# Layr-Labs/rust-kzg-bn254

Hardware: AMD Instinct MI355X
Metric: G1-MSM (scalar,point) pairs/s = 2^20 x KZG coeff-form commitments/s, 2^20-point SRS (higher is better)
Workload: dtype int32x9 (29-bit limbs, 64-bit accumulate); 1 GPU; G1 MSM 2^20 scalars (KZG::commit_coeff_form), scalars resident in HBM; step k commits buffer k mod 8 (8 distinct resident scalar sets, 256 MiB); pipeline_depth=2, steps_per_launch=1

## Files before the change

rust-kzg-bn254_amd/csrc/msm.hip:

```cpp
#include "engine.h"
#include <new>
#include "msm_kernels.h"
#include "host_msm_epilogue.h"
#include "host_pairing.h"

#include <algorithm>
#include <cstdlib>
#include <chrono>
#include <cstdio>
#include <cstring>
#include <type_traits>
#include <vector>

namespace kzg {

void MsmWorkspace::release() {
    DeviceBuffer* all[] = {&scalars, &bases, &bases_wire, &digits, &sorted, &count, &blockbase, &sort_tmp, &sort_key, &sort_small, &offs, &block_sums,
                           &head, &cont, &blob, &bucket, &chunkS, &chunkTmp, &chunkA, &out_wire};
    for (auto* b : all) b->release();
    if (pinned_out) { (void)hipHostFree(pinned_out); pinned_out = nullptr; }
    if (ev_ready) { for (auto& e : ev) (void)hipEventDestroy(e); ev_ready = false; }
    if (ev_done) { (void)hipEventDestroy(ev_done); ev_done = nullptr; }
    if (ev_sorted) { (void)hipEventDestroy(ev_sorted); ev_sorted = nullptr; }
}
// ... 127 lines not shown
    const Plan& p = L.p;
    MsmWorkspace& ws = L.ws;
    hipStream_t st = L.st;
    const uint32_t n_total = p.n * p.batch;
    KZG_HIP_TRY(L.ctx, hipMemsetAsync(ws.count.p, 0, (size_t)p.G * 4, st));
    hipLaunchKernelGGL(k_msm_digits, dim3((n_total + 255) / 256), dim3(256), 0, st, L.d_scalars, n_total, p.n, p.c, p.W, ws.digits.as<uint32_t>(), (uint32_t*)nullptr);
    KZG_MARK(1);
    if (p.sort_small) {
        const uint32_t entries = (uint32_t)p.entries(), ge = (uint32_t)((p.entries() + 255) / 256);
        KZG_HIP_TRY(L.ctx, hipMemsetAsync(ws.blockbase.p, 0, (size_t)p.G * 4, st));
        hipLaunchKernelGGL(k_sort_small_hist, dim3(ge), dim3(256), 0, st, ws.digits.as<uint32_t>(), entries, p.set_len, p.B, ws.count.as<uint32_t>());
        scan_counts(L);
        KZG_MARK(2);
        hipLaunchKernelGGL(k_sort_small_scatter, dim3(ge), dim3(256), 0, st, ws.digits.as<uint32_t>(), entries, p.n, p.set_len, p.B,
                           ws.offs.as<uint32_t>(), ws.blockbase.as<uint32_t>(), p.idx_stride, (uint32_t)p.W, ws.sorted.as<uint32_t>());
    } else {
        const size_t lds_bytes = (size_t)p.B * 4;
        hipLaunchKernelGGL(k_sort_hist, dim3(p.tiles), dim3(256), lds_bytes, st, ws.digits.as<uint32_t>(), p.set_len, p.tile_len,
                           p.tiles_per_set, p.B, ws.count.as<uint32_t>(), ws.blockbase.as<uint32_t>());
        scan_counts(L);
        KZG_MARK(2);
        hipLaunchKernelGGL(k_sort_scatter, dim3(p.tiles), dim3(256), lds_bytes, st, ws.digits.as<uint32_t>(), p.n, p.set_len, p.tile_len,
                           p.tiles_per_set, p.B, ws.offs.as<uint32_t>(), ws.blockbase.as<uint32_t>(), p.idx_stride,
                           (uint32_t)p.W, ws.sorted.as<uint32_t>());
    }
    KZG_MARK(3);
    return KZG_OK;
}

static int32_t enqueue_sort(const Launch& L, const PolyPtrs* poly_ptrs) {
    const Plan& p = L.p;
    kzg_ctx* ctx = L.ctx;
    MsmWorkspace& ws = L.ws;
    if (p.bitsum) {
        for (int i = 0; i <= 4; ++i) KZG_MARK(i);
        return KZG_OK;
    }
    { int32_t rc = set_sort_lds_attributes(ctx); if (rc != KZG_OK) return rc; }
    const bool stagger = p.tables && p.polys >= 2;
    if (stagger && ctx->last_sorted && ctx->last_sorted_stream != L.st) KZG_HIP_TRY(ctx, hipStreamWaitEvent(L.st, ctx->last_sorted, 0));
    KZG_MARK(0);
    const uint32_t clean_g = ws.count_zero_ptr == ws.count.p ? ws.count_zero_g : 0;
    ws.count_zero_g = 0;
    const int32_t rc = p.sort2 ? sort_two_level(L, poly_ptrs) : p.lean_sort ? sort_lean(L, clean_g) : sort_from_digits(L);
    if (rc != KZG_OK) return rc;
    KZG_MARK(4);
    if (p.tables) {
        if (!ws.ev_sorted) KZG_HIP_TRY(ctx, hipEventCreateWithFlags(&ws.ev_sorted, hipEventDisableTiming));
        KZG_HIP_TRY(ctx, hipEventRecord(ws.ev_sorted, L.st));
        ctx->last_sorted = ws.ev_sorted;
        ctx->last_sorted_stream = L.st;
    }
    return KZG_OK;
}

static int32_t enqueue_accumulate(const Launch& L) {
    const Plan& p = L.p;
    MsmWorkspace& ws = L.ws;
    if (!p.bitsum && !p.fused)
        dispatch<true, false>(!L.bases.identity_free, [&](auto identity_bases) {
            hipLaunchKernelGGL(k_msm_accumulate<decltype(identity_bases)::value>, dim3(p.nl / 256), dim3(256), 0, L.st, L.bases.points, ws.sorted.as<uint32_t>(),
                               ws.offs.as<uint32_t>(), p.G, ws.head.as<int32_t>(), (size_t)p.G, ws.cont.as<int32_t>(), (size_t)p.nl, p.idx_log, p.stride_adj);
        });
    KZG_MARK(5);
    return KZG_OK;
}

static int32_t reduce_bitsum(const Launch& L) {
    const Plan& p = L.p;
    dispatch<8, 16, 32>(p.bitsum_chunk, [&](auto chunk) {
        hipLaunchKernelGGL(k_bitsum_level1<decltype(chunk)::value>, dim3(p.bitsum_wg), dim3(256), 0, L.st, L.bases.points, L.bases.table_stride, L.d_scalars, p.n,
                           L.ws.chunkS.as<int32_t>());
    });
    KZG_MARK(6);
    hipLaunchKernelGGL(k_bitsum_level2, dim3(p.n_out), dim3(256), 0, L.st, L.ws.chunkS.as<int32_t>(), p.bitsum_wg, L.d_out);
    return KZG_OK;
}

static int32_t reduce_tables(const Launch& L) {
    const Plan& p = L.p;
    MsmWorkspace& ws = L.ws;
    const uint32_t G1 = p.G1(), G1p = p.G1p();
    int32_t* x1 = ws.chunkS.as<int32_t>();
    dispatch<true, false>(p.quad1, [&](auto quads) {
        using LG = std::conditional_t<decltype(quads)::value, QuadLanes, PairLanes>;
        if (p.fused)
            hipLaunchKernelGGL(k_msm_bucket_bits1_fused<LG>, dim3(G1), dim3(LG::THREADS), 0, L.st, L.bases.points, ws.sorted.as<uint32_t>(), ws.offs.as<uint32_t>(), p.B,
                               p.idx_log, p.stride_adj, G1, x1, (size_t)7 * G1, L.d_out);
        else
            hipLaunchKernelGGL(k_msm_bucket_bits1<LG>, dim3(G1), dim3(LG::THREADS), 0, L.st, ws.offs.as<uint32_t>(), p.B, p.nl, ws.head.as<int32_t>(), (size_t)p.G,
                               ws.cont.as<int32_t>(), (size_t)p.nl, G1, x1, (size_t)7 * G1, L.d_out);
    });
    KZG_MARK(6);
    if (p.polys && p.c == 7) {
        hipLaunchKernelGGL(k_batch_finish, dim3((p.polys + 63) / 64), dim3(64), 0, L.st, x1, (size_t)7 * G1, G1, L.d_out);
    } else if (G1 > 1) {
        const uint32_t waves2 = 7 * G1p;
        if (p.quad)
            hipLaunchKernelGGL(k_red_bits2q, dim3(waves2), dim3(256), 0, L.st, x1, (size_t)7 * G1, G1, G1p, L.d_out);
        else
            hipLaunchKernelGGL(k_red_bits2p, dim3((waves2 + 1) / 2), dim3(128), 0, L.st, x1, (size_t)7 * G1, G1, G1p, L.d_out);
    }
    return KZG_OK;
}

static int32_t reduce_generic(const Launch& L) {
    const Plan& p = L.p;
    MsmWorkspace& ws = L.ws;
    hipStream_t st = L.st;
    const uint32_t n_chunks = p.n_chunks(), n_windows = p.n_windows();
    const uint32_t gg = (p.G + 255) / 256;
    hipLaunchKernelGGL(k_msm_bucket_fin, dim3(gg), dim3(256), 0, st, ws.offs.as<uint32_t>(), p.G, p.nl, p.m, n_chunks, ws.head.as<int32_t>(), (size_t)p.G,
                       ws.cont.as<int32_t>(), (size_t)p.nl, ws.bucket.as<int32_t>(), (size_t)p.G);
    const uint32_t gc = (n_chunks + 255) / 256;
    KZG_MARK(6);
    hipLaunchKernelGGL(k_red_chunk_sums, dim3(gc), dim3(256), 0, st, ws.bucket.as<int32_t>(), (size_t)p.G, n_chunks, p.m,
                       ws.chunkS.as<int32_t>(), (size_t)n_chunks);
    hipLaunchKernelGGL(k_red_suffix_scan, dim3(n_windows), dim3(p.T), 0, st, ws.chunkS.as<int32_t>(), ws.chunkTmp.as<int32_t>(),
                       (size_t)n_chunks, p.T);
    hipLaunchKernelGGL(k_red_chunk_running, dim3(gc), dim3(256), 0, st, ws.bucket.as<int32_t>(), (size_t)p.G,
                       ws.chunkS.as<int32_t>(), (size_t)n_chunks, n_chunks, p.T, p.m, ws.chunkA.as<int32_t>());
    hipLaunchKernelGGL(k_red_window_sum, dim3(n_windows), dim3(p.T), 0, st, ws.chunkA.as<int32_t>(), (size_t)n_chunks, p.T,
                       L.d_out);
    return KZG_OK;
}

static int32_t enqueue_reduce(const Launch& L) {
    const int32_t rc = L.p.bitsum ? reduce_bitsum(L) : L.p.tables ? reduce_tables(L) : reduce_generic(L);
    if (rc != KZG_OK) return rc;
    KZG_MARK(7);
    return KZG_OK;
}
#undef KZG_MARK

static PlanContext plan_context(const kzg_ctx* ctx) {
    PlanContext pc;
    pc.msm_c_override = ctx->msm_c_override;
    pc.msm_seg_override = ctx->msm_seg_override;
    pc.reduction_lanes = ctx->reduction_lanes;
    pc.acc_wave_slots = ctx->acc_wave_slots;
    for (int sl = 0; sl < KZG_NUM_SLOTS; ++sl) pc.other_in_flight |= ctx->slot_pending[sl] != nullptr;
    return pc;
}

static int32_t msm_enqueue(kzg_ctx* ctx, MsmWorkspace& ws, hipStream_t st, const MsmBases& bases, const uint4* d_scalars, size_t n,
                           uint32_t batch, Pending* pend, uint32_t out_off = 0, uint32_t out_cap = MSM_MAX_OUT, uint32_t polys = 0,
                           const PolyPtrs* poly_ptrs = nullptr) {
    const Plan p = make_plan(plan_context(ctx), n, bases, batch, polys);
    {
        const char* error = nullptr;
        const int32_t rc = msm_plan_status(p, bases, polys, out_off, out_cap, &error);
        if (error) ctx->last_error = error;
        if (rc != KZG_OK) return rc;
    }
    DeviceBuffer* const buffers[WS_BUFFERS] = {&ws.digits, &ws.sorted, &ws.count, &ws.sort_tmp, &ws.sort_key, &ws.sort_small, &ws.blockbase, &ws.offs, &ws.block_sums,
                                               &ws.head, &ws.cont, &ws.bucket, &ws.chunkS, &ws.chunkTmp, &ws.chunkA};
    for (int i = 0; i < WS_BUFFERS; ++i) KZG_HIP_TRY(ctx, buffers[i]->reserve(p.bytes[i]));
    if (!ws.pinned_out) {
        KZG_HIP_TRY(ctx, hipHostMalloc(&ws.pinned_out, (size_t)MSM_MAX_OUT * 32 * 4 + MSM_MAX_PARTS * 4, hipHostMallocDefault));
        KZG_HIP_TRY(ctx, hipHostGetDevicePointer(&ws.pinned_out_dev, ws.pinned_out, 0));
    }
    const Launch L{ctx, ws, st, bases, d_scalars, p, reinterpret_cast<uint32_t*>(ws.pinned_out_dev) + (size_t)out_off * 32, ctx->profiling};
    if (L.prof && !ws.ev_ready) {
        for (auto& e : ws.ev) KZG_HIP_TRY(ctx, hipEventCreate(&e));
        ws.ev_ready = true;
    }
    int32_t rc;
    RoctxPhases phases;
    phases.begin(p.bitsum ? "kzg:msm:bit sums" : "kzg:msm:sort");
    if ((rc = enqueue_sort(L, poly_ptrs)) != KZG_OK) return rc;
    if (!p.bitsum) phases.begin("kzg:msm:accumulate");
    if ((rc = enqueue_accumulate(L)) != KZG_OK) return rc;
    if (!p.bitsum) phases.begin("kzg:msm:bucket reduction");
    if ((rc = enqueue_reduce(L)) != KZG_OK) return rc;
    phases.end();
// ... 281 lines not shown
```

rust-kzg-bn254_amd/csrc/msm_kernels.h:

```cpp
#pragma once
#include <hip/hip_runtime.h>
#include "curve_pair.h"
#include "curve_quad.h"
#include "naf.h"
#include "msm_limits.h"

namespace kzg {

__device__ __forceinline__ void latency_bound_kernel() {
#if !defined(KZG_NO_SETPRIO)
    __builtin_amdgcn_s_setprio(3);
#endif
}

constexpr uint32_t DIGIT_NONE = 0xFFFFFFFFu;

__global__ void __launch_bounds__(256)
k_msm_digits(const uint4* __restrict__ scalars, uint32_t n_total, uint32_t n, int c, int W, uint32_t* __restrict__ digits,
             uint32_t* __restrict__ count = nullptr ) {
    latency_bound_kernel();
    uint32_t j = blockIdx.x * blockDim.x + threadIdx.x;
    if (j >= n_total) return;
    const uint32_t msm = j / n, i = j - msm * n;
    uint4 lo = scalars[2 * (size_t)j], hi = scalars[2 * (size_t)j + 1];
    uint32_t w32[8] = {lo.x, lo.y, lo.z, lo.w, hi.x, hi.y, hi.z, hi.w};
    uint32_t k[8];
    fe_wire_to_canonical_words<FrParams>(k, w32);
    const uint32_t mask = (1u << c) - 1u, half = 1u << (c - 1);
    uint32_t carry = 0;
    for (int w = 0; w < W; ++w) {
        uint32_t raw = (k[0] & mask) + carry;
#pragma unroll
        for (int j = 0; j < 7; ++j) k[j] = (k[j] >> c) | (k[j + 1] << (32 - c));
        k[7] >>= c;
        uint32_t neg = raw > half;
        uint32_t mag = neg ? (1u << c) - raw : raw;
        carry = neg;
        uint32_t v = DIGIT_NONE;
        if (mag != 0) {
            v = (mag - 1) | (neg << 31);
            if (count) atomicAdd(&count[mag - 1], 1u);
        }
        digits[((size_t)msm * W + w) * n + i] = v;
    }
}


template <int T>
__device__ __forceinline__ uint32_t block_excl_scan(uint32_t v, uint32_t* total, uint32_t* lds ) {
    const int t = threadIdx.x;
    lds[t] = v;
    __syncthreads();
    for (int d = 1; d < T; d <<= 1) {
        uint32_t x = (t >= d) ? lds[t - d] : 0u;
        __syncthreads();
        lds[t] += x;
        __syncthreads();
    }
    uint32_t incl = lds[t];
    *total = lds[T - 1];
    __syncthreads();
    return incl - v;
}
__device__ __forceinline__ uint4 scan1_load(const uint32_t* __restrict__ count, uint32_t g, uint32_t hi) {
    if (g + 4 <= hi) return *reinterpret_cast<const uint4*>(count + g);
    uint4 v = make_uint4(0, 0, 0, 0);
    if (g < hi) v.x = count[g];
    if (g + 1 < hi) v.y = count[g + 1];
    if (g + 2 < hi) v.z = count[g + 2];
    return v;
}
template <bool LEAN>
__global__ void __launch_bounds__(SCAN1_THREADS)
k_scan_counts_1wg(uint32_t* __restrict__ count, uint32_t G, uint32_t* __restrict__ offs , uint32_t* __restrict__ cursor ) {
    latency_bound_kernel();
    __shared__ uint32_t wave_total[SCAN1_THREADS / 64];
    const uint32_t t = threadIdx.x, w = t >> 6, lane = t & 63;
    const uint32_t per_wave = (((G + SCAN1_THREADS / 64 - 1) / (SCAN1_THREADS / 64)) + 255u) & ~255u;
    const uint32_t lo = min(G, w * per_wave), hi = min(G, lo + per_wave);
    uint32_t s = 0;
    for (uint32_t g0 = lo; g0 < hi; g0 += 1024) {
        const uint32_t g = g0 + lane * 4;
        const uint4 a = scan1_load(count, g, hi), b = scan1_load(count, g + 256, hi), c = scan1_load(count, g + 512, hi), d = scan1_load(count, g + 768, hi);
        s += a.x + a.y + a.z + a.w + b.x + b.y + b.z + b.w + c.x + c.y + c.z + c.w + d.x + d.y + d.z + d.w;
    }
    for (int d = 32; d >= 1; d >>= 1) s += __shfl_xor(s, d, 64);
    if (lane == 0) wave_total[w] = s;
    __syncthreads();
// ... 983 lines not shown
__device__ __forceinline__ void bucket_partial_lanes(typename LG::Point& v, const BucketSpan& s, uint32_t k, const int32_t* __restrict__ head, size_t head_stride,
                                                     const int32_t* __restrict__ cont, size_t cont_stride, typename LG::Role role) {
    if (k == 0) { LG::load(v, head, head_stride, s.g, role); return; }
    LG::load(v, cont, cont_stride, bucket_cont_lane(s, k), role);
}
template <class LG>
__device__ __noinline__ void bucket_sum_heavy(typename LG::Point& tot, uint32_t g, uint32_t t1, uint32_t np, uint32_t long_run, uint32_t lane,
                                              const int32_t* __restrict__ head, size_t head_stride, const int32_t* __restrict__ cont, size_t cont_stride) {
    const uint32_t grp = lane / LG::LANES;
    const typename LG::Role role = LG::role(lane);
    BucketSpan h;
    h.g = g; h.t1 = t1; h.np = np; h.long_run = long_run != 0;
    typename LG::Point part;
    LG::set_inf(part);
    const uint32_t loads = (np + LG::GROUPS - 1) / LG::GROUPS;
#pragma unroll 1
    for (uint32_t step = 0; step < loads + LG::LOG_GROUPS; ++step) {
        typename LG::Point u;
        bool on;
        if (step < loads) {
            const uint32_t k = grp + LG::GROUPS * step;
            on = k < np;
            if (on) bucket_partial_lanes<LG>(u, h, k, head, head_stride, cont, cont_stride, role);
        } else {
            const uint32_t d = (LG::GROUPS / 2) >> (step - loads);
            LG::shfl_down(u, part, (int)(LG::LANES * d));
            on = grp < d;
        }
        if (on) {
            typename LG::Point r;
            LG::add(r, part, u, role);
            part = r;
        }
    }
    LG::shfl(tot, part, (int)(lane & (LG::LANES - 1)));
}
template <class LG>
__device__ __forceinline__ void bucket_sum_lanes(typename LG::Point& acc, const BucketSpan& s, uint32_t lane, typename LG::Role role, const int32_t* __restrict__ head,
                                                 size_t head_stride, const int32_t* __restrict__ cont, size_t cont_stride) {
    LG::set_inf(acc);
    const bool heavy = s.np > NP_SERIAL;
    if (!heavy) {
#pragma unroll 1
        for (uint32_t k = 0; k < s.np; ++k) {
            typename LG::Point v, r;
            bucket_partial_lanes<LG>(v, s, k, head, head_stride, cont, cont_stride, role);
            LG::add(r, acc, v, role);
            acc = r;
        }
    }
    unsigned long long todo = __ballot(heavy && (lane & (LG::LANES - 1)) == 0);
    while (todo) {
        const int src = __ffsll((long long)todo) - 1;
        todo &= todo - 1;
        typename LG::Point tot;
        bucket_sum_heavy<LG>(tot, __shfl(s.g, src, 64), __shfl(s.t1, src, 64), __shfl(s.np, src, 64), (uint32_t)__shfl((int)s.long_run, src, 64), lane,
                             head, head_stride, cont, cont_stride);
        if ((int)(lane & ~(LG::LANES - 1)) == src) acc = tot;
    }
}
template <class LG>
__global__ void __launch_bounds__(LG::THREADS) __attribute__((amdgpu_waves_per_eu(LG::WAVES, LG::WAVES)))
k_msm_bucket_bits1(const uint32_t* __restrict__ offs, uint32_t B, uint32_t nl, const int32_t* __restrict__ head, size_t head_stride,
                   const int32_t* __restrict__ cont, size_t cont_stride, uint32_t G1, int32_t* __restrict__ x1, size_t x_stride,
                   uint32_t* __restrict__ out_wire ) {
    latency_bound_kernel();
    __shared__ int32_t lds[LG::ZETA_LDS_WORDS];
    const uint32_t g = blockIdx.x, w = threadIdx.x >> 6, lane = threadIdx.x & 63, gp = w * LG::GROUPS + lane / LG::LANES;
    const typename LG::Role role = LG::role(lane);
    const uint32_t L = acc_seg_len(offs[B], nl);
    const uint32_t bkt = g * 64 + gp;
    BucketSpan s;
    s.g = bkt; s.t1 = 0; s.np = 0; s.long_run = false;
    if (bkt < B && L) s = bucket_span(offs, bkt, L);
    typename LG::Point v;
    bucket_sum_lanes<LG>(v, s, lane, role, head, head_stride, cont, cont_stride);
    LG::zeta64(v, lane, w, role, lds);
    const int zr = zeta_role(gp);
    if (zr < 0) return;
    if (G1 == 1) LG::store_wire(out_wire, (size_t)zr, v, role);
    else LG::store(x1, x_stride, (size_t)zr * G1 + g, v, role);
}
template <class LG>
__device__ __noinline__ void fused_heavy_bucket(typename LG::Point& tot, uint32_t hb, uint32_t he, uint32_t lane, const uint4* __restrict__ points,
                                                const uint32_t* __restrict__ sorted, uint32_t idx_log, uint32_t stride_adj) {
    const uint32_t grp = lane / LG::LANES;
    const typename LG::Role role = LG::role(lane);
    typename LG::Point part;
    LG::set_inf(part);
#pragma unroll 1
    for (uint32_t e = hb + grp; e < he; e += LG::GROUPS) {
        const uint32_t cur = sorted[e];
        const uint4* src = points + 4 * acc_point_index(cur & 0x7FFFFFFFu, idx_log, stride_adj) + LG::affine_half(role);
        const uint4 q0 = src[0], q1 = src[1];
        const uint32_t w32[8] = {q0.x, q0.y, q0.z, q0.w, q1.x, q1.y, q1.z, q1.w};
        int any = (q0.x | q0.y | q0.z | q0.w | q1.x | q1.y | q1.z | q1.w) != 0 ? 1 : 0;
        any |= pair_swap(any);
        if (!any) continue;
        Fq c;
        fe_unpack(c, w32);
        typename LG::Point r;
        LG::madd(r, part, c, cur >> 31, role);
        part = r;
    }
#pragma unroll 1
    for (int d = LG::GROUPS / 2; d >= 1; d >>= 1) {
        typename LG::Point u;
        LG::shfl_down(u, part, (int)LG::LANES * d);
        if (grp < (uint32_t)d) {
            typename LG::Point r;
            LG::add(r, part, u, role);
            part = r;
        }
    }
    LG::shfl(tot, part, (int)(lane & (LG::LANES - 1)));
}
template <class LG>
__global__ void __launch_bounds__(LG::THREADS) __attribute__((amdgpu_waves_per_eu(LG::WAVES, LG::WAVES)))
k_msm_bucket_bits1_fused(const uint4* __restrict__ points, const uint32_t* __restrict__ sorted, const uint32_t* __restrict__ offs, uint32_t B,
                         uint32_t idx_log, uint32_t stride_adj, uint32_t G1, int32_t* __restrict__ x1, size_t x_stride,
                         uint32_t* __restrict__ out_wire ) {
    latency_bound_kernel();
    __shared__ int32_t lds[LG::ZETA_LDS_WORDS];
    const uint32_t g = blockIdx.x, w = threadIdx.x >> 6, lane = threadIdx.x & 63, gp = w * LG::GROUPS + lane / LG::LANES;
    const typename LG::Role role = LG::role(lane);
    const uint32_t bkt = gp * G1 + g;
    uint32_t e = 0, end = 0;
    if (bkt < B) { e = offs[bkt]; end = offs[bkt + 1]; }
    const uint32_t hb = e, he = end;
    const bool heavy = end - e > LG::FUSED_HEAVY;
    if (heavy) end = e;
    typename LG::Point v;
    LG::set_inf(v);
    const uint32_t half = LG::affine_half(role);
    const uint32_t last = end ? end - 1 : 0;
    uint32_t ent = e < end ? sorted[e] : 0u;
    uint32_t ent1 = e < end ? sorted[e + 1 < end ? e + 1 : last] : 0u;
    const uint4* src = points + 4 * acc_point_index(ent & 0x7FFFFFFFu, idx_log, stride_adj) + half;
    uint4 q0 = make_uint4(0, 0, 0, 0), q1 = q0;
    if (e < end) { q0 = src[0]; q1 = src[1]; }
#pragma unroll 1
    for (; e < end; ++e) {
        const uint32_t cur = ent;
        const uint32_t w32[8] = {q0.x, q0.y, q0.z, q0.w, q1.x, q1.y, q1.z, q1.w};
        int any = (q0.x | q0.y | q0.z | q0.w | q1.x | q1.y | q1.z | q1.w) != 0 ? 1 : 0;
        ent = ent1;
        src = points + 4 * acc_point_index(ent & 0x7FFFFFFFu, idx_log, stride_adj) + half;
        q0 = src[0]; q1 = src[1];
        ent1 = sorted[e + 2 < end ? e + 2 : last];
        any |= pair_swap(any);
        if (!any) continue;
        Fq c;
        fe_unpack(c, w32);
        typename LG::Point r;
        LG::madd(r, v, c, cur >> 31, role);
        v = r;
    }
    unsigned long long todo = __ballot(heavy && (lane & (LG::LANES - 1)) == 0);
    while (todo) {
        const int src_lane = __ffsll((long long)todo) - 1;
        todo &= todo - 1;
        typename LG::Point tot;
        fused_heavy_bucket<LG>(tot, __shfl(hb, src_lane, 64), __shfl(he, src_lane, 64), lane, points, sorted, idx_log, stride_adj);
        if ((int)(lane & ~(LG::LANES - 1)) == src_lane) v = tot;
    }
    LG::zeta64(v, lane, w, role, lds);
// ... 221 lines not shown
```

rust-kzg-bn254_amd/csrc/msm_plan.h:

```cpp
#pragma once
#include <algorithm>
#include <cstddef>
#include <cstdint>
#include "../../include/kzg_bn254_mi355x.h"
#include "msm_limits.h"
#include "naf.h"

namespace kzg {

struct MsmBasesShape {
    uint32_t table_stride = 0;
    int c = 0;
    int W = 0;
    bool bitsum = false;
    bool naf = false;
};

struct PlanContext {
    int msm_c_override = 0;
    int msm_seg_override = 0;
    int reduction_lanes = 0;
    uint32_t acc_wave_slots = 3 * 1024;
    bool other_in_flight = false;
};

enum WsBuffer { WS_DIGITS, WS_SORTED, WS_COUNT, WS_SORT_TMP, WS_SORT_KEY, WS_SORT_SMALL, WS_BLOCKBASE, WS_OFFS, WS_BLOCK_SUMS, WS_HEAD, WS_CONT, WS_BUCKET,
                WS_CHUNK_S, WS_CHUNK_TMP, WS_CHUNK_A, WS_BUFFERS };

inline int ilog2_floor(size_t n) { int k = 0; while ((n >> (k + 1)) != 0) ++k; return k; }

struct Plan {
    uint32_t n;
    uint32_t batch;
    bool tables;
    bool naf;
    uint32_t polys;
    int c, W;
    uint32_t B;
    uint32_t sets;
    uint32_t G;
    uint32_t nl;
    uint32_t set_len;
    uint32_t tile_len, tiles_per_set, tiles;
    bool bitsum;
    bool fused;
    bool quad;
    bool alone = false;
    bool sort2;
    bool sort_small;
    uint32_t Hb, tile1, tiles1, tiles2cap;
    uint32_t T, m;
    uint32_t idx_stride, idx_log, stride_adj;
    int ND;
    bool lean_sort;
    bool quad1;
    int bitsum_chunk;
    uint32_t bitsum_wg;
    uint32_t n_out;
    size_t bytes[WS_BUFFERS];

    uint32_t G1() const { return B / 64; }
    uint32_t G1p() const { return (G1() + 63) / 64; }
    uint32_t n_windows() const { return (uint32_t)W * batch; }
    uint32_t n_chunks() const { return n_windows() * T; }
    uint32_t scan_blocks() const { return (G + SCAN_TILE - 1) / SCAN_TILE; }
    size_t entries() const { return (size_t)W * n * batch; }
};

inline int generic_window(size_t n, uint32_t batch) {
    int c = std::min(14, std::max(4, ilog2_floor(n) - 6));
    while (c < 16 && (size_t)((255 + c - 1) / c) * batch > MSM_MAX_OUT) ++c;
    return c;
}

inline int batch_bucket_bits(size_t poly_len) {
    if (poly_len < ((size_t)1 << 13)) return 7;
    if (poly_len < ((size_t)1 << 15)) return 13;
    if (poly_len < ((size_t)1 << 18)) return 15;
    return 16;
}

inline size_t msm_launch_len(const MsmBasesShape& bases) {
    if (bases.naf) return MSM_MAX_LAUNCH;
    if (bases.table_stride != 0 && (size_t)bases.W * bases.table_stride > ((size_t)1 << SORT2_IDX_BITS)) {
        size_t cpow = 1;
        while (((size_t)bases.W * cpow * 2) <= ((size_t)1 << SORT2_IDX_BITS)) cpow *= 2;
        if (cpow >= ((size_t)1 << 16)) return cpow;
    }
    return MSM_MAX_LAUNCH;
}

inline size_t msm_batch_capacity(size_t n) {
    if (n == 0) return 0;
    const int cb = batch_bucket_bits(n);
    return std::min<size_t>(std::min<size_t>(MSM_BATCH_POLYS_MAX, (size_t)65536 >> (cb - 1)), MSM_MAX_LAUNCH / n);
}

inline Plan bitsum_plan(size_t n) {
    Plan p{};
    p.n = (uint32_t)n; p.batch = 1; p.tables = true; p.bitsum = true; p.B = 64; p.G = 64; p.W = 255; p.c = 7;
    p.bitsum_chunk = n <= 512 ? 8 : n <= 2048 ? 16 : 32;
    p.bitsum_wg = (uint32_t)((n * (size_t)(256 / p.bitsum_chunk) + 63) / 64);
    p.n_out = (p.bitsum_wg + 63) / 64;
    p.bytes[WS_CHUNK_S] = (size_t)p.bitsum_wg * 36 * 4;
    return p;
}

inline Plan make_plan(const PlanContext& ctx, size_t n, const MsmBasesShape& bases, uint32_t batch, uint32_t polys = 0) {
    if (bases.bitsum && batch == 1 && !polys && n <= BITSUM_MAX_N) return bitsum_plan(n);
    Plan p{};
    p.n = (uint32_t)n;
    p.batch = batch;
    p.tables = bases.table_stride != 0;
    p.naf = p.tables && bases.naf;
    p.polys = p.naf && polys <= MSM_BATCH_POLYS_MAX ? polys : 0;
    p.quad = p.tables && !ctx.other_in_flight;
    if (ctx.reduction_lanes) p.quad = p.tables && ctx.reduction_lanes == 4;
    p.alone = !ctx.other_in_flight;
    int c;
    if (p.polys) {
        c = batch_bucket_bits(n / p.polys);
    } else if (p.tables) {
        c = bases.c;
        if (p.naf && c == 16 && p.alone && n < ((size_t)1 << 19)) c = 15;
    } else {
        c = ctx.msm_c_override;
        if (c == 0) c = generic_window(n, batch);
        c = std::min(16, std::max(2, c));
    }
    p.c = c;
    p.W = p.naf ? naf_max_digits(c + 1) : (255 + c - 1) / c;
    p.B = p.polys ? (c == 7 ? 64u * ((p.polys + 1u) & ~1u) : p.polys << (c - 1)) : 1u << (c - 1);
    p.sets = p.tables ? 1u : (uint32_t)p.W * batch;
    p.G = p.sets * p.B;
    const size_t entries_cap = (size_t)p.W * n * batch;
    const size_t entries = p.naf ? std::max<size_t>(1, (size_t)((double)n * 254.0 / (double)(c + 2))) : entries_cap;
    {
        const int L = ctx.msm_seg_override;
        size_t lanes;
        if (L > 0) {
            lanes = (entries + (size_t)L - 1) / (size_t)L;
        } else {
            const size_t lmin = entries >= ((size_t)1 << 21) ? 24 : 4;
            size_t slots = ctx.acc_wave_slots;
            if (ctx.other_in_flight || entries < ((size_t)1 << 23)) slots = slots / 3 * 2;
            if (entries < ((size_t)1 << 22)) slots = ctx.acc_wave_slots / 3;
            lanes = std::min<size_t>(slots * 64, (entries + lmin - 1) / lmin);
        }
        lanes = std::max<size_t>(256, (lanes + 255) / 256 * 256);
        p.nl = (uint32_t)std::min<size_t>(lanes, (size_t)1 << 24);
    }
    p.set_len = (uint32_t)(p.tables ? entries_cap : n);
    p.idx_stride = bases.table_stride; p.idx_log = 31; p.stride_adj = 0;
    if (p.tables && !p.naf && (size_t)p.W * bases.table_stride > ((size_t)1 << SORT2_IDX_BITS)) {
        int lg = ilog2_floor(n);
        if (((size_t)1 << lg) < n) ++lg;
        if (((size_t)p.W << lg) <= ((size_t)1 << SORT2_IDX_BITS) && ((size_t)1 << lg) <= bases.table_stride) {
            p.idx_log = (uint32_t)lg; p.idx_stride = 1u << lg; p.stride_adj = bases.table_stride - p.idx_stride;
        }
    }
    size_t tile = std::max<size_t>(4096, 2 * (size_t)p.B);
    while (tile < p.set_len && ((size_t)p.set_len + tile - 1) / tile * p.sets > 1024) tile *= 2;
    p.tile_len = (uint32_t)tile;
    p.tiles_per_set = (uint32_t)(((size_t)p.set_len + tile - 1) / tile);
    p.tiles = p.tiles_per_set * p.sets;
    {
        const bool lds_fits = (size_t)p.B * 4 <= SORT1_MAX_LDS;
        p.sort_small = !p.naf && entries < ((size_t)1 << 18);
        const bool can2 = p.tables && (p.c - 1 > SORT2_LO_BITS || p.polys) && (p.B >> SORT2_LO_BITS) <= SORT2_MAX_BINS &&
                          (p.naf ? (size_t)NAF_POSITIONS * p.idx_stride < ((size_t)1 << 31)
                                 : (size_t)p.W * p.idx_stride <= ((size_t)1 << SORT2_IDX_BITS));
        p.sort2 = !p.sort_small && can2 && (entries >= ((size_t)1 << 18) || !lds_fits || p.naf);
        if (!p.sort2 && !lds_fits) p.sort_small = true;
        p.Hb = p.sort2 ? (p.B >> SORT2_LO_BITS) : 0;
        p.tile1 = n >= ((size_t)1 << 19) ? 2048 : 1024;
        if (p.naf) {
            p.tile1 = 512;
            if (p.polys) p.tile1 = 2048;
        }
        p.tiles1 = (uint32_t)((n + p.tile1 - 1) / p.tile1);
        p.tiles2cap = (uint32_t)(entries_cap / SORT2_CHUNK + p.Hb + 1);
    }
    p.T = std::min<uint32_t>(p.B, RED_T);
    p.m = p.B / p.T;
    p.ND = p.c + 1 >= 16 ? NAF_DIGITS : 32;
    p.lean_sort = !p.sort2 && p.sort_small && p.tables && batch == 1 && p.G == p.B && p.G <= SCAN1_MAX;
    p.fused = p.tables && !p.naf && (double)entries_cap <= 2.5 * (double)p.B;
    p.quad1 = p.quad && (p.fused || p.G1() <= 512 || ctx.reduction_lanes == 4);
    p.n_out = !p.tables ? p.n_windows() : p.polys && p.c == 7 ? p.polys : p.G1() == 1 ? 7 : 13 * p.G1p();

    size_t* by = p.bytes;
    by[WS_SORTED] = entries_cap * 4;
    by[WS_COUNT] = (size_t)p.G * 4 + 16;
    if (p.sort2) {
        by[WS_SORT_TMP] = entries_cap * 4;
        if (p.naf) {
            by[WS_SORT_KEY] = entries_cap + 16;
            by[WS_DIGITS] = (size_t)n * p.ND * 4;
        }
        by[WS_SORT_SMALL] = ((size_t)3 * (p.Hb + 1) + p.tiles2cap) * 4 + 64;
        by[WS_BLOCKBASE] = std::max((size_t)p.tiles1 * p.Hb, (size_t)p.tiles2cap * SORT2_LO) * 4;
    } else {
        by[WS_DIGITS] = entries_cap * 4;
        by[WS_BLOCKBASE] = p.sort_small ? (size_t)p.G * 4 : (size_t)p.tiles * p.B * 4;
    }
    by[WS_OFFS] = ((size_t)p.G + 1) * 4 + 16;
    by[WS_BLOCK_SUMS] = (size_t)SCAN_TILE * 4;
    by[WS_HEAD] = (size_t)p.G * 36 * 4;
    by[WS_CONT] = (size_t)p.nl * 36 * 4;
#ifdef KZG_ACC_STAMPS
    by[WS_CONT] += (size_t)(p.nl / 64) * 64;
#endif
    if (p.tables) {
        by[WS_CHUNK_S] = (size_t)7 * p.G1() * 36 * 4;
    } else {
        by[WS_BUCKET] = (size_t)p.G * 36 * 4;
        by[WS_CHUNK_S] = by[WS_CHUNK_TMP] = by[WS_CHUNK_A] = (size_t)p.n_chunks() * 36 * 4;
    }
    return p;
}

inline int32_t msm_plan_status(const Plan& p, const MsmBasesShape& bases, uint32_t polys, uint32_t out_off, uint32_t out_cap, const char** error) {
    *error = nullptr;
    if (p.batch == 0 || (p.batch > 1 && bases.table_stride != 0)) return KZG_ERR_INVALID_ARG;
    if (polys && (!bases.naf || p.n % polys != 0 || polys > MSM_BATCH_POLYS_MAX)) return KZG_ERR_INVALID_ARG;
    if (p.bitsum) return out_cap < p.n_out || out_off + p.n_out > MSM_MAX_OUT ? KZG_ERR_INVALID_ARG : KZG_OK;
    if (p.polys && p.B > 65536) return KZG_ERR_INVALID_ARG;
    if (!p.tables && p.n_windows() > MSM_MAX_OUT) return KZG_ERR_INVALID_ARG;
    if (p.G > SCAN1_MAX && p.scan_blocks() > SCAN_TILE) return KZG_ERR_INVALID_ARG;
    if (p.tables && p.G1() > 1 && 13 * p.G1p() > MSM_MAX_OUT) return KZG_ERR_INVALID_ARG;
    if (p.n_out > out_cap || out_off + p.n_out > MSM_MAX_OUT) {
        *error = "MSM result points exceed this launch's window of the result buffer";
        return KZG_ERR_INVALID_ARG;
    }
    return KZG_OK;
}

}
```

Measured before the change: 967.2 million pairs/s.

## Add row/column bucket reduction path for table MSM with pair lanes

Adds a two-kernel path that first writes each bucket sum to a bucket buffer, then reduces 4096-bucket units by summing 64 rows and 64 columns with chained adds and a small tree. The column sums feed the zeta64 bit-weighting and the row sums go into an extra slot, so the per-bucket weighting is split across row and column decomposition. It replaces the single fused bucket_bits1 pass for non-fused, non-quad plans whose G1 is a multiple of 64. This costs an extra bucket buffer round trip through HBM and one more launch, and it writes identity points into unused slots.

Result: slower. 921.5 million pairs/s (-4.7%).

```diff
diff --git a/rust-kzg-bn254_amd/csrc/msm.hip b/rust-kzg-bn254_amd/csrc/msm.hip
--- a/rust-kzg-bn254_amd/csrc/msm.hip
+++ b/rust-kzg-bn254_amd/csrc/msm.hip
@@ -233,15 +233,23 @@
     MsmWorkspace& ws = L.ws;
     const uint32_t G1 = p.G1(), G1p = p.G1p();
     int32_t* x1 = ws.chunkS.as<int32_t>();
-    dispatch<true, false>(p.quad1, [&](auto quads) {
-        using LG = std::conditional_t<decltype(quads)::value, QuadLanes, PairLanes>;
-        if (p.fused)
-            hipLaunchKernelGGL(k_msm_bucket_bits1_fused<LG>, dim3(G1), dim3(LG::THREADS), 0, L.st, L.bases.points, ws.sorted.as<uint32_t>(), ws.offs.as<uint32_t>(), p.B,
-                               p.idx_log, p.stride_adj, G1, x1, (size_t)7 * G1, L.d_out);
-        else
-            hipLaunchKernelGGL(k_msm_bucket_bits1<LG>, dim3(G1), dim3(LG::THREADS), 0, L.st, ws.offs.as<uint32_t>(), p.B, p.nl, ws.head.as<int32_t>(), (size_t)p.G,
-                               ws.cont.as<int32_t>(), (size_t)p.nl, G1, x1, (size_t)7 * G1, L.d_out);
-    });
+    if (p.rowcol) {
+        using LG = PairLanes;
+        hipLaunchKernelGGL(k_msm_bucket_sums<LG>, dim3(G1), dim3(LG::THREADS), 0, L.st, ws.offs.as<uint32_t>(), p.B, p.nl, ws.head.as<int32_t>(), (size_t)p.G,
+                           ws.cont.as<int32_t>(), (size_t)p.nl, ws.bucket.as<int32_t>(), (size_t)p.G);
+        hipLaunchKernelGGL(k_msm_rowcol<LG>, dim3(rowcol_workgroups(p.B)), dim3(ROWCOL_CHAINS * LG::LANES), 0, L.st, ws.bucket.as<int32_t>(), (size_t)p.G, G1, x1,
+                           (size_t)7 * G1);
+    } else {
+        dispatch<true, false>(p.quad1, [&](auto quads) {
+            using LG = std::conditional_t<decltype(quads)::value, QuadLanes, PairLanes>;
+            if (p.fused)
+                hipLaunchKernelGGL(k_msm_bucket_bits1_fused<LG>, dim3(G1), dim3(LG::THREADS), 0, L.st, L.bases.points, ws.sorted.as<uint32_t>(), ws.offs.as<uint32_t>(),
+                                   p.B, p.idx_log, p.stride_adj, G1, x1, (size_t)7 * G1, L.d_out);
+            else
+                hipLaunchKernelGGL(k_msm_bucket_bits1<LG>, dim3(G1), dim3(LG::THREADS), 0, L.st, ws.offs.as<uint32_t>(), p.B, p.nl, ws.head.as<int32_t>(), (size_t)p.G,
+                                   ws.cont.as<int32_t>(), (size_t)p.nl, G1, x1, (size_t)7 * G1, L.d_out);
+        });
+    }
     KZG_MARK(6);
     if (p.polys && p.c == 7) {
         hipLaunchKernelGGL(k_batch_finish, dim3((p.polys + 63) / 64), dim3(64), 0, L.st, x1, (size_t)7 * G1, G1, L.d_out);
diff --git a/rust-kzg-bn254_amd/csrc/msm_kernels.h b/rust-kzg-bn254_amd/csrc/msm_kernels.h
--- a/rust-kzg-bn254_amd/csrc/msm_kernels.h
+++ b/rust-kzg-bn254_amd/csrc/msm_kernels.h
@@ -4,6 +4,7 @@
 #include "curve_quad.h"
 #include "naf.h"
 #include "msm_limits.h"
+#include "msm_rowcol.h"
 
 namespace kzg {
 
@@ -1153,6 +1154,72 @@
     else LG::store(x1, x_stride, (size_t)zr * G1 + g, v, role);
 }
 template <class LG>
+__global__ void __launch_bounds__(LG::THREADS) __attribute__((amdgpu_waves_per_eu(LG::WAVES, LG::WAVES)))
+k_msm_bucket_sums(const uint32_t* __restrict__ offs, uint32_t B, uint32_t nl, const int32_t* __restrict__ head, size_t head_stride,
+                  const int32_t* __restrict__ cont, size_t cont_stride, int32_t* __restrict__ bucket, size_t bucket_stride) {
+    latency_bound_kernel();
+    const uint32_t w = threadIdx.x >> 6, lane = threadIdx.x & 63, gp = w * LG::GROUPS + lane / LG::LANES;
+    const typename LG::Role role = LG::role(lane);
+    const uint32_t L = acc_seg_len(offs[B], nl);
+    const uint32_t bkt = blockIdx.x * 64 + gp;
+    BucketSpan s;
+    s.g = bkt; s.t1 = 0; s.np = 0; s.long_run = false;
+    if (bkt < B && L) s = bucket_span(offs, bkt, L);
+    typename LG::Point v;
+    bucket_sum_lanes<LG>(v, s, lane, role, head, head_stride, cont, cont_stride);
+    if (bkt < B) LG::store(bucket, bucket_stride, bkt, v, role);
+}
+template <class LG>
+__global__ void __launch_bounds__(ROWCOL_CHAINS * LG::LANES) __attribute__((amdgpu_waves_per_eu(LG::WAVES, LG::WAVES)))
+k_msm_rowcol(const int32_t* __restrict__ bucket, size_t bucket_stride, uint32_t G1, int32_t* __restrict__ x1, size_t x_stride) {
+    static_assert(LG::GROUPS % ROWCOL_PARTS == 0, "the chains of a line sit in one wave");
+    latency_bound_kernel();
+    __shared__ int32_t lds[LG::ZETA_LDS_WORDS];
+    __shared__ int32_t cols[4 * NL * 64];
+    const uint32_t unit = rowcol_unit(blockIdx.x), kind = rowcol_kind(blockIdx.x);
+    const uint32_t w = threadIdx.x >> 6, lane = threadIdx.x & 63, chain = threadIdx.x / LG::LANES;
+    const typename LG::Role role = LG::role(lane);
+    const uint32_t line = rowcol_line(chain), part = rowcol_part(chain);
+    typename LG::Point acc;
+    LG::set_inf(acc);
+#pragma unroll 1
+    for (uint32_t step = 0; step < ROWCOL_CHAIN + ROWCOL_TREE_STEPS; ++step) {
+        typename LG::Point u;
+        bool on = true;
+        if (step < ROWCOL_CHAIN) {
+            LG::load(u, bucket, bucket_stride, rowcol_bucket(kind, unit, chain, step), role);
+        } else {
+            const uint32_t t = step - ROWCOL_CHAIN;
+            LG::shfl_down(u, acc, (int)(LG::LANES * rowcol_tree_span(t)));
+            on = rowcol_tree_adds(part, t);
+        }
+        if (on) {
+            typename LG::Point r;
+            LG::add(r, acc, u, role);
+            acc = r;
+        }
+    }
+    if (kind == ROWCOL_ROWS) {
+        if (part == 0) LG::store(x1, x_stride, rowcol_row_slot(G1, unit, line), acc, role);
+        return;
+    }
+    {
+        typename LG::Point inf;
+        LG::set_inf(inf);
+        for (uint32_t i = chain; i < ROWCOL_IDENTITY_SLOTS; i += ROWCOL_CHAINS) LG::store(x1, x_stride, rowcol_identity_slot(G1, unit, i), inf, role);
+    }
+    if (part == 0) LG::store(cols, 64, line, acc, role);
+    __syncthreads();
+    if (w >= LG::THREADS / 64) return;
+    typename LG::Point v;
+    const uint32_t gp = threadIdx.x / LG::LANES;
+    LG::load(v, cols, 64, gp, role);
+    LG::zeta64(v, lane, w, role, lds);
+    const int zr = zeta_role(gp);
+    if (zr >= 0 && zr < 6) LG::store(x1, x_stride, rowcol_bit_slot(G1, unit, (uint32_t)zr), v, role);
+}
+
+template <class LG>
 __device__ __noinline__ void fused_heavy_bucket(typename LG::Point& tot, uint32_t hb, uint32_t he, uint32_t lane, const uint4* __restrict__ points,
                                                 const uint32_t* __restrict__ sorted, uint32_t idx_log, uint32_t stride_adj) {
     const uint32_t grp = lane / LG::LANES;
diff --git a/rust-kzg-bn254_amd/csrc/msm_plan.h b/rust-kzg-bn254_amd/csrc/msm_plan.h
--- a/rust-kzg-bn254_amd/csrc/msm_plan.h
+++ b/rust-kzg-bn254_amd/csrc/msm_plan.h
@@ -54,6 +54,7 @@
     int ND;
     bool lean_sort;
     bool quad1;
+    bool rowcol;
     int bitsum_chunk;
     uint32_t bitsum_wg;
     uint32_t n_out;
@@ -187,6 +188,7 @@
     p.lean_sort = !p.sort2 && p.sort_small && p.tables && batch == 1 && p.G == p.B && p.G <= SCAN1_MAX;
     p.fused = p.tables && !p.naf && (double)entries_cap <= 2.5 * (double)p.B;
     p.quad1 = p.quad && (p.fused || p.G1() <= 512 || ctx.reduction_lanes == 4);
+    p.rowcol = p.tables && !p.fused && !p.bitsum && !p.polys && !p.quad && !p.quad1 && p.G1() != 0 && p.G1() % 64 == 0;
     p.n_out = !p.tables ? p.n_windows() : p.polys && p.c == 7 ? p.polys : p.G1() == 1 ? 7 : 13 * p.G1p();
 
     size_t* by = p.bytes;
@@ -213,6 +215,7 @@
 #endif
     if (p.tables) {
         by[WS_CHUNK_S] = (size_t)7 * p.G1() * 36 * 4;
+        if (p.rowcol) by[WS_BUCKET] = (size_t)p.G * 36 * 4;
     } else {
         by[WS_BUCKET] = (size_t)p.G * 36 * 4;
         by[WS_CHUNK_S] = by[WS_CHUNK_TMP] = by[WS_CHUNK_A] = (size_t)p.n_chunks() * 36 * 4;
diff --git a/rust-kzg-bn254_amd/csrc/msm_rowcol.h b/rust-kzg-bn254_amd/csrc/msm_rowcol.h
--- /dev/null
+++ b/rust-kzg-bn254_amd/csrc/msm_rowcol.h
@@ -0,0 +1,39 @@
+#pragma once
+#include <cstdint>
+
+#if defined(__HIPCC__)
+#define KZG_ROWCOL_HD __host__ __device__ __forceinline__
+#else
+#define KZG_ROWCOL_HD inline
+#endif
+
+namespace kzg {
+
+constexpr uint32_t ROWCOL_UNIT = 4096;
+constexpr uint32_t ROWCOL_LINE = 64;
+constexpr uint32_t ROWCOL_CHAIN = 16;
+constexpr uint32_t ROWCOL_PARTS = ROWCOL_LINE / ROWCOL_CHAIN;
+constexpr uint32_t ROWCOL_TREE_STEPS = 2;
+constexpr uint32_t ROWCOL_CHAINS = ROWCOL_LINE * ROWCOL_PARTS;
+enum RowColKind : uint32_t { ROWCOL_ROWS = 0, ROWCOL_COLS = 1 };
+static_assert(ROWCOL_PARTS == 1u << ROWCOL_TREE_STEPS && ROWCOL_CHAIN * ROWCOL_PARTS == ROWCOL_LINE && ROWCOL_LINE * ROWCOL_LINE == ROWCOL_UNIT, "rowcol schedule");
+
+KZG_ROWCOL_HD uint32_t rowcol_workgroups(uint32_t B) { return 2 * (B / ROWCOL_UNIT); }
+KZG_ROWCOL_HD uint32_t rowcol_unit(uint32_t wg) { return wg >> 1; }
+KZG_ROWCOL_HD uint32_t rowcol_kind(uint32_t wg) { return wg & 1u; }
+KZG_ROWCOL_HD uint32_t rowcol_line(uint32_t chain) { return chain / ROWCOL_PARTS; }
+KZG_ROWCOL_HD uint32_t rowcol_part(uint32_t chain) { return chain % ROWCOL_PARTS; }
+KZG_ROWCOL_HD uint32_t rowcol_bucket(uint32_t kind, uint32_t unit, uint32_t chain, uint32_t step) {
+    const uint32_t line = rowcol_line(chain), pos = ROWCOL_PARTS * step + rowcol_part(chain);
+    return unit * ROWCOL_UNIT + (kind == ROWCOL_ROWS ? line * ROWCOL_LINE + pos : pos * ROWCOL_LINE + line);
+}
+KZG_ROWCOL_HD uint32_t rowcol_tree_span(uint32_t t) { return (ROWCOL_PARTS / 2) >> t; }
+KZG_ROWCOL_HD bool rowcol_tree_adds(uint32_t part, uint32_t t) { return part < rowcol_tree_span(t); }
+KZG_ROWCOL_HD uint32_t rowcol_row_slot(uint32_t G1, uint32_t unit, uint32_t line) { return 6 * G1 + unit * ROWCOL_LINE + line; }
+KZG_ROWCOL_HD uint32_t rowcol_bit_slot(uint32_t G1, uint32_t unit, uint32_t k) { return k * G1 + unit * ROWCOL_LINE; }
+constexpr uint32_t ROWCOL_IDENTITY_SLOTS = 6 * (ROWCOL_LINE - 1);
+KZG_ROWCOL_HD uint32_t rowcol_identity_slot(uint32_t G1, uint32_t unit, uint32_t i) {
+    return (i / (ROWCOL_LINE - 1)) * G1 + unit * ROWCOL_LINE + 1 + i % (ROWCOL_LINE - 1);
+}
+
+}
```
